# MohammadJohari/myslam

Hardware: AMD Instinct MI355X
Metric: ray.samples/s (render+bwd) (higher is better)
Workload: dtype f32; 1 GPU; BASELINE configs[1]: Replica room0 (synthetic), 4096 rays x 64 samples (56+8); mapping iteration: sample + render fwd + loss + bwd (planes+decoders), no optimiser; rays_of_the_job=4096, rays_this_rank=4096, samples_per_ray=64, plane_bytes=27147008, planes_layout=channels_last, parallelism=single GPU, launch=hipGraph replay of the captured iteration

## Files before the change

myslam_amd/csrc/eslam_scatter.hip:

```cpp
#include <mutex>
#include <type_traits>
#include "eslam_decode_tile.h"
#include "eslam_dec_reduce.h"
#include "eslam_ray_order_dev.h"

typedef float float2_t __attribute__((ext_vector_type(2)));

__global__ __launch_bounds__(1024) void ray_order_kernel(const float* __restrict__ rays_o,
                                                         const float* __restrict__ rays_d, int R,
                                                         int* __restrict__ perm, int key_bits, const int n_order,
                                                         float* __restrict__ clear, const long long clear_words) {
    extern __shared__ __attribute__((aligned(16))) unsigned hist[];
    if ((int)blockIdx.x >= n_order) {
        ray_clear_block(clear, clear_words, (int)blockIdx.x - n_order, (int)gridDim.x - n_order);
        return;
    }
    ray_order_block(rays_o, rays_d, R, perm, key_bits, (int)blockIdx.x, hist);
}

#define FIX_SCALE 17592186044416.0f
#define FIX_LIMIT 262144.0f
struct ShadowOff { int64_t o[NPL]; };
constexpr int SC_NT = 512;
constexpr int GZ_WP = 20;
template <bool RENDER, bool DET, int SPT = 4, bool GZ = false>
__global__ __launch_bounds__(SC_NT) void scatter_sort_kernel(const PlaneSet planes, const Bound bnd,
                                                          const float* __restrict__ rays_o,
                                                          const float* __restrict__ rays_d,
                                                          const float* __restrict__ z_vals,
                                                          const int* __restrict__ perm, int R, int S,
                                                          const float* __restrict__ g_feat, int bundle, int nbundles,
                                                          long long* __restrict__ shadow,
                                                          const ShadowOff shoff, const DecReduceArgs red, const int red_blocks,
                                                          const float* __restrict__ gz_w1_sdf, const float* __restrict__ gz_w1_rgb) {
    constexpr int NT = SC_NT;
    static_assert(!GZ || (RENDER && !DET), "GZ: the float render path only");
    constexpr int BM = SPT * NT;
    constexpr int CH = WAVE * SPT;
    static_assert(SPT == 2 || SPT == 4, "samples per thread");
    constexpr int SLOT_BITS = (BM == 1024) ? 10 : 11;
    constexpr unsigned SLOT_MASK = BM - 1;
    static_assert(BM == 1024 || BM == 2048, "bundle size");
    __shared__ __attribute__((aligned(16))) unsigned lds_raw[6 * BM];
    __shared__ __attribute__((aligned(16))) float gz_w[GZ ? ESLAM_C_DIM * GZ_WP : 4];
    __shared__ __attribute__((aligned(16))) float gz_a[GZ ? NT : 4];
    float4_t* const sw = (float4_t*)lds_raw;
    unsigned* const sxy = lds_raw + 4 * BM;
    int* const sgrow = (int*)(lds_raw + 5 * BM);
    unsigned* const cnt = lds_raw;
    unsigned* const swsum = lds_raw + 2 * BM;
    int* const sbox = (int*)(lds_raw + 2 * BM + 64);
    unsigned* const skey = lds_raw;
    unsigned* const txy = lds_raw + BM;
    float* const ttm = (float*)(lds_raw + 2 * BM + 128);
    float* const ttM = (float*)(lds_raw + 3 * BM + 128);
    int* const trow = (int*)(lds_raw + 4 * BM + 128);
    constexpr unsigned PAD_XY = 0xFFFFFFFFu;
    const int lane = threadIdx.x & 63, wave = threadIdx.x >> 6;
    const int hx = lane >> 5, c = lane & 31;

    if (red_blocks > 0 && (int)blockIdx.x < red_blocks) {
        if ((int)blockIdx.x < 2 * DEC_RED_COLBLOCKS)
            dec_grad_reduce_block<NT>(red, blockIdx.x % DEC_RED_COLBLOCKS, blockIdx.x / DEC_RED_COLBLOCKS, (float*)lds_raw);
        return;
    }
    const int bid = (int)blockIdx.x - red_blocks;
    bool plane_major = false;
    if (RENDER && perm) {
        const float* fan = (const float*)(perm + (size_t)ESLAM_RAY_ORDERS * R);
        const float f0 = fan[0], f1 = fan[1], f2 = fan[2];
        const float second = fmaxf(fminf(f0, f1), fminf(fmaxf(f0, f1), f2));
        plane_major = second >= 1.4f;
    }
    int bidx, pi;
    if (plane_major) { bidx = bid % nbundles; pi = bid / nbundles; }
    else { pi = bid % NPL; bidx = bid / NPL; }
    if (bidx >= nbundles || pi >= NPL) return;
    const int d = pi / 6, o = (pi % 6) >> 1, lvl = pi & 1;
    const eslam_plane_t& P = planes.p[pi];
    float gz_wv = 0.0f;
    if (GZ) gz_wv = (d ? gz_w1_rgb : gz_w1_sdf)[(threadIdx.x >> 5) * ESLAM_FEAT + lvl * ESLAM_C_DIM + (threadIdx.x & 31)];
    static_assert(!GZ || NT == ESLAM_HIDDEN * ESLAM_C_DIM, "one element of the slice per thread");
    const int pw = P.w, ph = P.h;
    const int psy = (int)P.stride_y, psx = (int)P.stride_x, psc = (int)P.stride_c;
    float* __restrict__ grad = P.grad;
    const int64_t npts = RENDER ? (int64_t)R * S : (int64_t)R;
    const int nunits = RENDER ? R : (int)((npts + 63) / 64);
    const int per = RENDER ? S : 64;
    const int u0 = bidx * bundle;
    const int nu = min(bundle, nunits - u0);
    const int n = nu * per;

    bool swap = false;
    if (threadIdx.x == 0) { sbox[0] = 0x7FFFFFFF; sbox[1] = -1; sbox[2] = 0x7FFFFFFF; sbox[3] = -1; }
    __syncthreads();

    AxisCoord cax[SPT], cay[SPT];
    int cpt[SPT];
    int bx0 = 0x7FFFFFFF, bx1 = -1, by0 = 0x7FFFFFFF, by1 = -1;
#pragma unroll
    for (int k = 0; k < SPT; ++k) {
        const int slot = threadIdx.x + k * NT;
        cpt[k] = -1;
        if (slot < n) {
            const int ui = u0 + slot / per, s = slot % per;
            const int unit = (RENDER && perm) ? perm[(size_t)o * R + ui] : ui;
            const int64_t pt = RENDER ? (int64_t)unit * S + s : (int64_t)unit * 64 + s;
            if (pt < npts) {
                float x, y, z;
                if (RENDER) {
                    const float zz = z_vals[pt];
                    x = rays_o[unit * 3 + 0] + rays_d[unit * 3 + 0] * zz;
                    y = rays_o[unit * 3 + 1] + rays_d[unit * 3 + 1] * zz;
                    z = rays_o[unit * 3 + 2] + rays_d[unit * 3 + 2] * zz;
                } else {
                    x = z_vals[pt * 3 + 0]; y = z_vals[pt * 3 + 1]; z = z_vals[pt * 3 + 2];
                }
                x = norm_coord(x, bnd.lo[0], bnd.hi[0]);
                y = norm_coord(y, bnd.lo[1], bnd.hi[1]);
                z = norm_coord(z, bnd.lo[2], bnd.hi[2]);
                cax[k] = axis_coord((o == 2) ? y : x, pw);
                cay[k] = axis_coord((o == 0) ? y : z, ph);
                cpt[k] = (int)pt;
                bx0 = min(bx0, cax[k].i0); bx1 = max(bx1, cax[k].i0);
                by0 = min(by0, cay[k].i0); by1 = max(by1, cay[k].i0);
            }
        }
    }
    if (GZ) gz_w[(threadIdx.x & 31) * GZ_WP + (threadIdx.x >> 5)] = gz_wv;
    bx0 = wave_min_i(bx0); bx1 = wave_max_i(bx1);
    by0 = wave_min_i(by0); by1 = wave_max_i(by1);
    if (lane == 0) {
        atomicMin(&sbox[0], bx0); atomicMax(&sbox[1], bx1);
        atomicMin(&sbox[2], by0); atomicMax(&sbox[3], by1);
    }
    __syncthreads();
    const int bxmin = sbox[0], bxmax = sbox[1], bymin = sbox[2], bymax = sbox[3];
    __syncthreads();
    if (bxmax < 0) return;
    swap = (bymax - bymin) > (bxmax - bxmin);
    const int mmin = swap ? bymin : bxmin, mext = (swap ? bymax : bxmax) - mmin + 2;
    const int Mmin = swap ? bxmin : bymin, Mext = (swap ? bxmax : bymax) - Mmin + 1;
    const bool counting = (int64_t)mext * Mext <= 4 * BM;
    if (counting) {
        constexpr int WPT = 2 * BM / NT;
        for (int i = threadIdx.x; i < 2 * BM; i += NT) cnt[i] = 0u;
        __syncthreads();
        unsigned loc[SPT], tick[SPT];
#pragma unroll
        for (int k = 0; k < SPT; ++k) {
            loc[k] = 0; tick[k] = 0;
            if (cpt[k] >= 0) {
                const int im = swap ? cay[k].i0 : cax[k].i0, iM = swap ? cax[k].i0 : cay[k].i0;
                loc[k] = (unsigned)((iM - Mmin) * mext + (im - mmin));
                const unsigned sh = (loc[k] & 1u) * 16u;
                tick[k] = (atomicAdd(&cnt[loc[k] >> 1], 1u << sh) >> sh) & 0xFFFFu;
            }
        }
        __syncthreads();
        unsigned w[WPT], local = 0;
#pragma unroll
        for (int j = 0; j < WPT; ++j) {
            w[j] = cnt[threadIdx.x * WPT + j];
            local += (w[j] & 0xFFFFu) + (w[j] >> 16);
        }
        const unsigned incl = wave_incl_sum_u(local);
        if (lane == WAVE - 1) swsum[wave] = incl;
        __syncthreads();
        unsigned run = incl - local, nvalid = 0;
        for (int wv = 0; wv < NT / WAVE; ++wv) {
            if (wv < wave) run += swsum[wv];
            nvalid += swsum[wv];
        }
#pragma unroll
        for (int j = 0; j < WPT; ++j) {
            const unsigned lo16 = w[j] & 0xFFFFu, hi16 = w[j] >> 16;
            cnt[threadIdx.x * WPT + j] = run | ((run + lo16) << 16);
            run += lo16 + hi16;
        }
        __syncthreads();
        unsigned pos[SPT];
#pragma unroll
        for (int k = 0; k < SPT; ++k) pos[k] = ((cnt[loc[k] >> 1] >> ((loc[k] & 1u) * 16u)) & 0xFFFFu) + tick[k];
        __syncthreads();
#pragma unroll
        for (int k = 0; k < SPT; ++k) {
            if (cpt[k] >= 0) {
                const AxisCoord& am = swap ? cay[k] : cax[k];
                const AxisCoord& aM = swap ? cax[k] : cay[k];
                const unsigned q = pos[k];
                sxy[q] = ((unsigned)(cay[k].i0 * psy + cax[k].i0 * psx) << 2) | (unsigned)(am.i1 > am.i0) |
                         ((unsigned)(aM.i1 > aM.i0) << 1);
                sw[q] = (float4_t){(1.0f - am.t) * (1.0f - aM.t), (1.0f - am.t) * aM.t, am.t * (1.0f - aM.t), am.t * aM.t};
                sgrow[q] = cpt[k];
            }
        }
        for (int i = (int)nvalid + threadIdx.x; i < BM; i += NT) {
            sxy[i] = PAD_XY;
            sw[i] = (float4_t){0.f, 0.f, 0.f, 0.f};
            sgrow[i] = 0;
        }
        __syncthreads();
    } else {
#pragma unroll
    for (int k = 0; k < SPT; ++k) {
        const int slot = threadIdx.x + k * NT;
        unsigned key = 0xFFFFFFFFu;
        if (cpt[k] >= 0) {
            const AxisCoord& am = swap ? cay[k] : cax[k];
            const AxisCoord& aM = swap ? cax[k] : cay[k];
            const int cell = aM.i0 * (swap ? ph : pw) + am.i0;
            key = ((unsigned)cell << SLOT_BITS) | (unsigned)slot;
            txy[slot] = ((unsigned)(cay[k].i0 * psy + cax[k].i0 * psx) << 2) | (unsigned)(am.i1 > am.i0) |
                        ((unsigned)(aM.i1 > aM.i0) << 1);
            ttm[slot] = am.t;
            ttM[slot] = aM.t;
            trow[slot] = cpt[k];
        }
        skey[slot] = key;
    }
    __syncthreads();

    {
        const int wbase = wave * CH;
        for (int k = 2; k <= BM; k <<= 1) {
            for (int j = k >> 1; j > 0; j >>= 1) {
                if (j >= CH) {
                    __syncthreads();
#pragma unroll
                    for (int t = 0; t < SPT / 2; ++t) {
                        const int p = threadIdx.x + t * NT;
                        const int i = ((p & ~(j - 1)) << 1) | (p & (j - 1));
                        const int l = i | j;
                        const unsigned a = skey[i], b2 = skey[l];
                        if ((a > b2) == ((i & k) == 0)) { skey[i] = b2; skey[l] = a; }
                    }
                    __syncthreads();
                } else {
#pragma unroll
                    for (int t = 0; t < SPT / 2; ++t) {
                        const int p = lane + t * WAVE;
                        const int i = wbase + (((p & ~(j - 1)) << 1) | (p & (j - 1)));
                        const int l = i | j;
                        const unsigned a = skey[i], b2 = skey[l];
                        if ((a > b2) == ((i & k) == 0)) { skey[i] = b2; skey[l] = a; }
                    }
                    WAVE_SYNC();
                }
            }
        }
    }
    __syncthreads();
    unsigned pxy[SPT];
    float ptm[SPT], ptM[SPT];
    int prow[SPT];
#pragma unroll
    for (int k = 0; k < SPT; ++k) {
        const unsigned key = skey[threadIdx.x + k * NT];
        const bool valid = key != 0xFFFFFFFFu;
        const int slot = key & SLOT_MASK;
        pxy[k] = valid ? txy[slot] : PAD_XY;
        ptm[k] = valid ? ttm[slot] : 0.f;
        ptM[k] = valid ? ttM[slot] : 0.f;
        prow[k] = valid ? trow[slot] : 0;
    }
    __syncthreads();
#pragma unroll
    for (int k = 0; k < SPT; ++k) {
        const int q = threadIdx.x + k * NT;
        const bool valid = pxy[k] != PAD_XY;
        sxy[q] = pxy[k];
        sw[q] = valid ? (float4_t){(1.0f - ptm[k]) * (1.0f - ptM[k]), (1.0f - ptm[k]) * ptM[k], ptm[k] * (1.0f - ptM[k]),
                                   ptm[k] * ptM[k]}
                      : (float4_t){0.f, 0.f, 0.f, 0.f};
        sgrow[q] = prow[k];
    }
    __syncthreads();
    }

    const char* __restrict__ gcol = GZ ? (const char*)(g_feat + (size_t)d * (size_t)npts * 16)
                                       : (const char*)(g_feat + d * 64 + lvl * 32);
    unsigned cur_xy = PAD_XY;
    unsigned last_xy = PAD_XY;
    typedef typename std::conditional<DET, long long, float>::type acc_t;
    acc_t acc0 = 0, acc1 = 0;
    bool det_bad = false;
    const int e0 = wave * CH;

    const unsigned lane_off = (unsigned)(c * psc) << 2;
    const unsigned dm_bytes = (unsigned)(swap ? psy : psx) << 2, dM_bytes = (unsigned)(swap ? psx : psy) << 2;
    char* __restrict__ gbytes = DET ? (char*)(shadow + shoff.o[pi]) : (char*)grad;
    float* const gz_as = gz_a + (GZ ? wave * WAVE : 0);
    auto flush = [&](bool lower_half_only) {
        if (cur_xy != PAD_XY) {
            acc_t f0 = acc0, f1 = acc1;
            if (GZ) {
                gz_as[lane] = (float)acc0;
                WAVE_SYNC();
                const float4_t* const A = (const float4_t*)(gz_as + hx * 32);
                unsigned wrow = (unsigned)(c * GZ_WP);
                asm volatile("" : "+v"(wrow));
                const float4_t* const Wc = (const float4_t*)(gz_w + wrow);
                float r0 = 0.0f, r1 = 0.0f;
#pragma unroll
                for (int jj = 0; jj < 4; ++jj) {
                    const float4_t a0 = A[jj], a1 = A[4 + jj], wv = Wc[jj];
#pragma unroll
                    for (int i = 0; i < 4; ++i) { r0 += wv[i] * a0[i]; r1 += wv[i] * a1[i]; }
                    if (jj & 1) asm volatile("" : "+v"(r0), "+v"(r1));
                }
                WAVE_SYNC();
                f0 = (acc_t)r0;
                f1 = (acc_t)r1;
            }
            const unsigned o0 = (cur_xy & ~3u) + lane_off + ((cur_xy & 1u) & (unsigned)hx) * dm_bytes;
            const unsigned o1 = o0 + ((cur_xy >> 1) & 1u) * dM_bytes;
            if (DET) {
                if (!lower_half_only || hx == 0) {
                    atomicAdd((unsigned long long*)(gbytes + 2 * (size_t)o0), (unsigned long long)f0);
                    atomicAdd((unsigned long long*)(gbytes + 2 * (size_t)o1), (unsigned long long)f1);
                    if (det_bad) {
                        atomicAdd((float*)((char*)grad + o0), __builtin_nanf(""));
                        atomicAdd((float*)((char*)grad + o1), __builtin_nanf(""));
                    }
                }
            } else if (!lower_half_only || hx == 0) {
                atomicAdd((float*)(gbytes + o0), (float)f0);
                atomicAdd((float*)(gbytes + o1), (float)f1);
            }
        }
    };

    struct Rec { unsigned xy; int row; unsigned long long fresh, adjacent; };
    auto fetch = [&](int blk, unsigned prev_last) {
        Rec r;
        const int e = e0 + blk * WAVE + lane;
        r.xy = sxy[e];
        r.row = sgrow[e] * (GZ ? 64 : 512);
        unsigned prev = __shfl_up(r.xy, 1, WAVE);
        if (lane == 0) prev = prev_last;
        const bool fresh = r.xy != prev;
        const bool adj = fresh && r.xy != PAD_XY && prev != PAD_XY && (prev & 1u) && (r.xy & ~3u) == (prev & ~3u) + dm_bytes;
        r.fresh = __ballot(fresh);
        r.adjacent = __ballot(adj);
        return r;
    };
    constexpr int WALK_N = 8;
    const float2_t* const wlane = (const float2_t*)sw + hx;
    const float* const wlane1 = (const float*)sw + (lane >> 4);
    const __amdgpu_buffer_rsrc_t grsrc = __builtin_amdgcn_make_buffer_rsrc((void*)gcol, 0, GZ ? (int)((unsigned)npts * 64u) : (int)((unsigned)npts * 512u - (unsigned)(d * 64 + lvl * 32) * 4u), 0x00020000);
    const int cvoff = GZ ? (lane & 15) * 4 : c * 4;
#define LOAD_HALF(buf, rec, half)                                                             \
    _Pragma("unroll") for (int t = 0; t < WALK_N; ++t) {                                      \
        const int rowb = __builtin_amdgcn_readlane((rec).row, (half) * WALK_N + t);           \
        buf[t] = __builtin_bit_cast(float, __builtin_amdgcn_raw_buffer_load_b32(grsrc, cvoff, rowb, 0)); \
    }
#define WALK_HALF(buf, rec, half, ebase)                                                      \
    _Pragma("unroll") for (int t = 0; t < WALK_N; ++t) {                                      \
        const int idx = (half) * WALK_N + t;                                                  \
        float2_t w2 = {0.f, 0.f};                                                             \
        if (GZ) w2[0] = wlane1[4 * ((ebase) + idx)];                                          \
        else w2 = wlane[2 * ((ebase) + idx)];                                                 \
        if (((idx < 32 ? fresh_lo : fresh_hi) >> (idx & 31)) & 1u) {      \
            if (((idx < 32 ? adj_lo : adj_hi) >> (idx & 31)) & 1u) {                          \
                 \
                flush(true);                                                                  \
                const acc_t s0 = __shfl_xor(acc0, 32, WAVE), s1 = __shfl_xor(acc1, 32, WAVE); \
                acc0 = hx ? (acc_t)0 : s0;                                                    \
                acc1 = (hx || GZ) ? (acc_t)0 : s1;                                            \
                if (DET) {             \
                    const int carried_bad = __shfl_xor((int)det_bad, 32, WAVE);               \
                    det_bad = !hx && carried_bad;                                             \
                }                                                                             \
            } else {                                                                          \
                flush(false);                                                                 \
                det_bad = false;                                                              \
                acc0 = 0;                                                                     \
                acc1 = 0;                                                                     \
            }                                                                                 \
            cur_xy = (unsigned)__builtin_amdgcn_readlane((int)(rec).xy, idx);                 \
        }                                                                                     \
        const float g = buf[t];         \
        if (DET) {                                                                            \
            const float t0_ = g * w2[0], t1_ = g * w2[1];                                     \
            det_bad = det_bad || !(fabsf(t0_) < FIX_LIMIT) || !(fabsf(t1_) < FIX_LIMIT);      \
            acc0 += (acc_t)__float2ll_rn(t0_ * FIX_SCALE);                                    \
            acc1 += (acc_t)__float2ll_rn(t1_ * FIX_SCALE);                                    \
        } else if (GZ) {                                                                      \
            acc0 += (acc_t)(g * w2[0]);                                                       \
        } else {                                                                              \
            acc0 += (acc_t)(g * w2[0]);                                                       \
            acc1 += (acc_t)(g * w2[1]);                                                       \
        }                                                                                     \
    }

    const int nblk = CH / WAVE;
    const int ngrp = WAVE / WALK_N;
    float ga[WALK_N], gb[WALK_N];
    Rec rec = fetch(0, PAD_XY);
    LOAD_HALF(ga, rec, 0)
#pragma unroll 1
    for (int blk = 0; blk < nblk; ++blk) {
        if ((unsigned)__builtin_amdgcn_readfirstlane((int)rec.xy) == PAD_XY) break;
        last_xy = (unsigned)__builtin_amdgcn_readlane((int)rec.xy, WAVE - 1);
        Rec nxt = rec;
        if (blk + 1 < nblk) nxt = fetch(blk + 1, last_xy);
        const int ebase = e0 + blk * WAVE;
        const unsigned fresh_lo = (unsigned)__builtin_amdgcn_readfirstlane((int)(unsigned)rec.fresh);
        const unsigned fresh_hi = (unsigned)__builtin_amdgcn_readfirstlane((int)(unsigned)(rec.fresh >> 32));
        const unsigned adj_lo = (unsigned)__builtin_amdgcn_readfirstlane((int)(unsigned)rec.adjacent);
        const unsigned adj_hi = (unsigned)__builtin_amdgcn_readfirstlane((int)(unsigned)(rec.adjacent >> 32));
#pragma unroll
        for (int g2 = 0; g2 < ngrp; g2 += 2) {
            LOAD_HALF(gb, rec, g2 + 1)
            WALK_HALF(ga, rec, g2, ebase)
            if (g2 + 2 < ngrp) {
                LOAD_HALF(ga, rec, g2 + 2)
            } else if (blk + 1 < nblk) {
                LOAD_HALF(ga, nxt, 0)
            }
            WALK_HALF(gb, rec, g2 + 1, ebase)
        }
        rec = nxt;
    }
#undef LOAD_HALF
#undef WALK_HALF
    flush(false);
}

__global__ __launch_bounds__(256) void scatter_fixed_to_float_kernel(float* __restrict__ grad, long long* __restrict__ shadow,
                                                                     int64_t n) {
    for (int64_t i = (int64_t)blockIdx.x * 256 + threadIdx.x; i < n; i += (int64_t)gridDim.x * 256) {
        const long long v = shadow[i];
        if (v != 0) {
            grad[i] += (float)((double)v * (1.0 / 17592186044416.0));
            shadow[i] = 0;
        }
    }
}

int eslam_scatter_v2_init();

static int ray_order_launch(const char* who, const float* rays_o, const float* rays_d, int R, int32_t* perm, void* clear,
                            int64_t clear_bytes, eslam_stream_t stream) {
    if (ray_order_check_args(who, rays_o, rays_d, R, perm, clear, clear_bytes)) return 1;
    if (R <= 0 && clear_bytes == 0) return 0;
    hipStream_t st = (hipStream_t)stream;
    if (int rc = eslam_scatter_v2_init()) return rc;
    const int key_bits = ray_order_key_bits(R);
    const int n_clear = ray_clear_blocks(clear_bytes);
    const int n_order = ray_order_blocks(R);
    hipLaunchKernelGGL(ray_order_kernel, dim3(n_order + n_clear), dim3(1024), ray_order_lds_bytes(key_bits), st,
                       rays_o, rays_d, R, perm, key_bits, n_order, (float*)clear, (long long)(clear_bytes >> 2));
    return eslam_check_launch("ray_order_kernel");
}

extern "C" int eslam_ray_order(const float* rays_o, const float* rays_d, int R, int32_t* perm, eslam_stream_t stream) {
    if (R <= 0) return 0;
    return ray_order_launch("eslam_ray_order", rays_o, rays_d, R, perm, nullptr, 0, stream);
}

extern "C" int eslam_ray_order_clear(const float* rays_o, const float* rays_d, int R, int32_t* perm, void* clear_ptr,
                                     int64_t clear_bytes, eslam_stream_t stream) {
    return ray_order_launch("eslam_ray_order_clear", rays_o, rays_d, R, perm, clear_ptr, clear_bytes, stream);
}

#define SC_SMALL_WGS 192
static int scatter_bundle_size(int per, int nunits, int* bm_out) {
    int bm = 2048;
    if (!eslam_deterministic()) {
        const int big = 2048 / per;
        const int nb = big > 0 ? (nunits + big - 1) / big : nunits;
        bm = (nb * NPL <= SC_SMALL_WGS && 1024 / per >= 1) ? 1024 : 2048;
    }
    *bm_out = bm;
    return bm / per;
}

extern "C" int eslam_scatter_bundle_samples(int64_t n, int S, int render) {
    if (n <= 0 || (render && (S <= 0 || S > 256))) return 0;
    int bm = 0;
    (void)scatter_bundle_size(render ? S : 64, render ? (int)n : (int)((n + 63) / 64), &bm);
    return bm;
}

bool eslam_scatter_can_reduce(bool render) {
    return render && !eslam_deterministic();
}

int eslam_scatter_v2(const eslam_plane_t* planes, const Bound& bnd, const float* rays_o, const float* rays_d,
                     const float* z_or_pts, int64_t R, int S, bool render, const float* g_feat, const int* perm,
                     hipStream_t st, const DecReduceArgs* red, const eslam_decoders_t* gz_dec) {
    PlaneSet ps;
    for (int i = 0; i < NPL; ++i) {
        ps.p[i] = planes[i];

    }
    const int64_t N = render ? R * S : R;
    const int nunits = render ? (int)R : (int)((N + 63) / 64);
    if (gz_dec && (!render || eslam_deterministic())) {
        eslam_set_error("scatter: the rank-16 path serves the float render mode only");
        return 1;
    }
    static_assert(2 * 64 <= 512 && ESLAM_HIDDEN * 4 == 64, "the rank-16 rows' offsets lie inside the N * 512 limit checked below");
    if (gz_dec && (N * 128 >= ((int64_t)1 << 32) - 256 || N * 64 > INT32_MAX)) {
        eslam_set_error("scatter: %lld points exceed the 32-bit offset range of the 16-wide gradient rows", (long long)N);
        return 1;
    }
    if (N * 512 >= ((int64_t)1 << 32)) {
        eslam_set_error("scatter: %lld points exceed the 32-bit offset range of the feature-gradient buffer (8.3 M): split "
                        "the batch", (long long)N);
        return 1;
    }
    for (int i = 0; i < NPL; ++i) {
        const int64_t extent = (ESLAM_C_DIM - 1) * planes[i].stride_c + (int64_t)(planes[i].h - 1) * planes[i].stride_y +
                               (int64_t)(planes[i].w - 1) * planes[i].stride_x + 1;
        if (extent >= ((int64_t)1 << 30)) {
            eslam_set_error("scatter: plane %d spans %lld elements, limit 2^30", i, (long long)extent);
            return 1;
        }
    }
    const int per = render ? S : 64;
    int bm;
    const int bundle = scatter_bundle_size(per, nunits, &bm);
    for (int i = 0; i < NPL; ++i)
        if ((int64_t)planes[i].w * planes[i].h >= ((1 << 21) - 2)) {
            eslam_set_error("scatter: plane %d has %d x %d cells, limit 2^21", i, planes[i].h, planes[i].w);
            return 1;
        }
    const int nbundles = (nunits + bundle - 1) / bundle;
    dim3 grid(nbundles * NPL);
    DecReduceArgs red_args = {};
    int red_blocks = 0;
    if (red) {
        if (!eslam_scatter_can_reduce(render)) {
            eslam_set_error("scatter: cannot carry the decoder-gradient reduction in this mode");
            return 1;
        }
        red_args = *red;
        red_blocks = (2 * DEC_RED_COLBLOCKS + 7) / 8 * 8;
        grid.x += red_blocks;
    }
#define LAUNCH_SC(RD, PERM, SS, ...)                                                                                      \
    hipLaunchKernelGGL((scatter_sort_kernel<RD, false, ##__VA_ARGS__>), grid, dim3(SC_NT), 0, st, ps, bnd, rays_o, rays_d, z_or_pts, \
                       PERM, (int)R, SS, g_feat, bundle, nbundles, (long long*)nullptr, ShadowOff{}, red_args, red_blocks, \
                       gz_dec ? gz_dec->w1 : nullptr, gz_dec ? gz_dec->cw1 : nullptr)
    if (eslam_deterministic()) {
        ShadowOff so;
        int64_t total = 0;
        for (int i = 0; i < NPL; ++i) {
            const int64_t numel = (int64_t)ESLAM_C_DIM * planes[i].h * planes[i].w;
            const int64_t extent = (ESLAM_C_DIM - 1) * planes[i].stride_c + (int64_t)(planes[i].h - 1) * planes[i].stride_y +
                                   (int64_t)(planes[i].w - 1) * planes[i].stride_x + 1;
            if (extent != numel) {
                eslam_set_error("scatter (deterministic mode): plane %d is not dense", i);
                return 1;
            }
            so.o[i] = total;
            total += numel;
        }
        constexpr int MAXDEV = 64;
        static long long* shadows[MAXDEV];
        static int64_t shadow_ns[MAXDEV];
        static std::mutex shadow_mu;
        int devi = 0;
        if (hipGetDevice(&devi) != hipSuccess || devi < 0 || devi >= MAXDEV) {
            eslam_set_error("scatter (deterministic mode): no usable current device");
            return 2;
        }
        long long* shadow;
        {
            std::lock_guard<std::mutex> lk(shadow_mu);
            if (shadow_ns[devi] < total) {
                hipStreamCaptureStatus cs = hipStreamCaptureStatusNone;
                (void)hipStreamIsCapturing(st, &cs);
                if (cs != hipStreamCaptureStatusNone) {
                    eslam_set_error("scatter (deterministic mode): run one eager iteration before capturing a graph");
                    return 1;
                }
                long long* fresh = nullptr;
                if (hipMalloc(&fresh, (size_t)total * 8) != hipSuccess || hipMemset(fresh, 0, (size_t)total * 8) != hipSuccess) {
                    eslam_set_error("scatter (deterministic mode): cannot allocate the %lld-element shadow", (long long)total);
                    return 2;
                }
                shadows[devi] = fresh;
                shadow_ns[devi] = total;
            }
            shadow = shadows[devi];
        }
        if (render)
            hipLaunchKernelGGL((scatter_sort_kernel<true, true>), grid, dim3(SC_NT), 0, st, ps, bnd, rays_o, rays_d,
                               z_or_pts, perm, (int)R, S, g_feat, bundle, nbundles, shadow, so, DecReduceArgs{}, 0, nullptr, nullptr);
        else
            hipLaunchKernelGGL((scatter_sort_kernel<false, true>), grid, dim3(SC_NT), 0, st, ps, bnd, rays_o, rays_d,
                               z_or_pts, (const int*)nullptr, (int)R, 64, g_feat, bundle, nbundles, shadow, so,
                               DecReduceArgs{}, 0, nullptr, nullptr);
        if (int rc = eslam_check_launch("scatter_sort_kernel<det>")) return rc;
        for (int i = 0; i < NPL; ++i) {
            const int64_t numel = (int64_t)ESLAM_C_DIM * planes[i].h * planes[i].w;
            hipLaunchKernelGGL(scatter_fixed_to_float_kernel, dim3((unsigned)((numel + 255) / 256 < 2048 ? (numel + 255) / 256 : 2048)),
                               dim3(256), 0, st, planes[i].grad, shadow + so.o[i], numel);
        }
        return eslam_check_launch("scatter_fixed_to_float_kernel");
    }
    if (gz_dec) {
        if (bm == 1024) LAUNCH_SC(true, perm, S, 2, true);
        else LAUNCH_SC(true, perm, S, 4, true);
    } else if (render) {
        if (bm == 1024) LAUNCH_SC(true, perm, S, 2);
        else LAUNCH_SC(true, perm, S);
    } else {
        if (bm == 1024) LAUNCH_SC(false, (const int*)nullptr, 64, 2);
        else LAUNCH_SC(false, (const int*)nullptr, 64);
    }
#undef LAUNCH_SC
    return eslam_check_launch("scatter_sort_kernel");
}

bool eslam_planes_channels_last(const eslam_plane_t* planes, int first, int count);
int eslam_validate_planes(const eslam_plane_t* planes, int first, int count);

int eslam_scatter_v2_init() {
    static bool done = false;
    if (done) return 0;
    if (hipFuncSetAttribute((const void*)ray_order_kernel, hipFuncAttributeMaxDynamicSharedMemorySize,
                            ORD_CELLS * (int)sizeof(unsigned)) != hipSuccess) {
        eslam_set_error("scatter: hipFuncSetAttribute(MaxDynamicSharedMemorySize) failed");
        return 2;
    }
    done = true;
    return 0;
}
```

Measured before the change: 1.138 billion ray.samples/s.

## Restructure GZ scatter walk to process four samples per step across lane quads

Adds a dedicated GZ path in the plane-gradient scatter kernel. Each lane group of 16 now handles one of four consecutive samples, with per-sample row indices and float4 corner weights. Partial sums are combined with permlane16/permlane32 swaps before the shared-memory projection and the atomics. The aim is to cut the number of serial walk steps and per-sample loads per wave in the compressed-gradient path, at the cost of more complex per-nibble cell-closing logic and reliance on gfx950 permlane-swap instructions.

```diff
diff --git a/myslam_amd/csrc/eslam_scatter.hip b/myslam_amd/csrc/eslam_scatter.hip
--- a/myslam_amd/csrc/eslam_scatter.hip
+++ b/myslam_amd/csrc/eslam_scatter.hip
@@ -291,28 +291,124 @@
     const unsigned dm_bytes = (unsigned)(swap ? psy : psx) << 2, dM_bytes = (unsigned)(swap ? psx : psy) << 2;
     char* __restrict__ gbytes = DET ? (char*)(shadow + shoff.o[pi]) : (char*)grad;
     float* const gz_as = gz_a + (GZ ? wave * WAVE : 0);
+    if constexpr (GZ) {
+        int wl = lane;
+        asm volatile("" : "+v"(wl));
+        const int s = wl >> 4, whx = wl >> 5, wc = wl & 31;
+        const unsigned wlane_off = (unsigned)(wc * psc) << 2;
+        const int up1 = ((wl + WAVE - 1) & (WAVE - 1)) << 2;
+        float2_t alo = {0.f, 0.f}, ahi = {0.f, 0.f};
+        auto flush4 = [&](const bool lower_half_only) {
+            if (cur_xy == PAD_XY) return;
+            float x0 = alo[0], y0 = alo[1], x1 = ahi[0], y1 = ahi[1];
+            asm volatile("s_nop 1\n\tv_permlane16_swap_b32 %0, %1" : "+v"(x0), "+v"(y0));
+            asm volatile("s_nop 1\n\tv_permlane16_swap_b32 %0, %1" : "+v"(x1), "+v"(y1));
+            float r0 = x0 + y0, r1 = x1 + y1;
+            asm volatile("s_nop 1\n\tv_permlane32_swap_b32 %0, %1" : "+v"(r0), "+v"(r1));
+            gz_as[wl] = r0 + r1;
+            WAVE_SYNC();
+            const float4_t* const A = (const float4_t*)(gz_as + whx * 32);
+            unsigned wrow = (unsigned)(wc * GZ_WP);
+            asm volatile("" : "+v"(wrow));
+            const float4_t* const Wc = (const float4_t*)(gz_w + wrow);
+            float f0 = 0.0f, f1 = 0.0f;
+#pragma unroll
+            for (int jj = 0; jj < 4; ++jj) {
+                const float4_t v0 = A[jj], v1 = A[4 + jj], wv = Wc[jj];
+#pragma unroll
+                for (int i = 0; i < 4; ++i) { f0 += wv[i] * v0[i]; f1 += wv[i] * v1[i]; }
+                if ((jj & 1) || SPT == 2) asm volatile("" : "+v"(f0), "+v"(f1));
+            }
+            WAVE_SYNC();
+            const unsigned o0 = (cur_xy & ~3u) + wlane_off + ((cur_xy & 1u) & (unsigned)whx) * dm_bytes;
+            const unsigned o1 = o0 + ((cur_xy >> 1) & 1u) * dM_bytes;
+            if (!lower_half_only || whx == 0) {
+                atomicAdd((float*)(gbytes + o0), f0);
+                atomicAdd((float*)(gbytes + o1), f1);
+            }
+        };
+        struct Rec4 { unsigned xy; unsigned long long fresh, adjacent; };
+        auto fetch4 = [&](int blk, unsigned prev_last) {
+            Rec4 r;
+            r.xy = sxy[e0 + blk * WAVE + wl];
+            unsigned prev = (unsigned)__builtin_amdgcn_ds_bpermute(up1, (int)r.xy);
+            if (wl == 0) prev = prev_last;
+            const bool fresh = r.xy != prev;
+            const bool adj = fresh && r.xy != PAD_XY && prev != PAD_XY && (prev & 1u) && (r.xy & ~3u) == (prev & ~3u) + dm_bytes;
+            r.fresh = __ballot(fresh);
+            r.adjacent = __ballot(adj);
+            return r;
+        };
+        auto close_cell = [&](const Rec4& rec, const int e, const int kk, const bool carry, const float4_t w4, float& g) {
+            const float gk = (s < kk) ? g : 0.f;
+            g = (s < kk) ? 0.f : g;
+            alo += gk * w4.xy;
+            ahi += gk * w4.zw;
+            flush4(carry);
+            alo = carry ? ahi : (float2_t){0.f, 0.f};
+            ahi = (float2_t){0.f, 0.f};
+            cur_xy = (unsigned)__builtin_amdgcn_readlane((int)rec.xy, e + kk);
+        };
+        constexpr int WALK_Q = 4;
+        const __amdgpu_buffer_rsrc_t grsrc4 = __builtin_amdgcn_make_buffer_rsrc((void*)gcol, 0, (int)((unsigned)npts * 64u), 0x00020000);
+        const int j4 = (wl & 15) * 4;
+        const int* const rlane = sgrow + s;
+        const float4_t* const wlane4 = sw + s;
+#define LOAD_Q(buf, eb, grp)                                                                  \
+    _Pragma("unroll") for (int t = 0; t < WALK_Q; ++t) {                                      \
+        const int row = rlane[(eb) + 4 * ((grp) * WALK_Q + t)];                               \
+        buf[t] = __builtin_bit_cast(float, __builtin_amdgcn_raw_buffer_load_b32(grsrc4, (row << 6) + j4, 0, 0)); \
+    }
+#define WALK_Q4(buf, rec, grp, eb)                                                            \
+    _Pragma("unroll") for (int t = 0; t < WALK_Q; ++t) {                                      \
+        const int st = (grp) * WALK_Q + t;                                                    \
+        const float4_t w4 = wlane4[(eb) + 4 * st];                                            \
+        const unsigned nib = ((st < 8 ? fresh_lo : fresh_hi) >> (4 * (st & 7))) & 15u;        \
+        float g = buf[t];                                                                     \
+        for (unsigned m = nib; __builtin_expect(m != 0u, 0); m &= m - 1u) {                   \
+            const int kk = __builtin_ctz(m);                                                  \
+            close_cell(rec, 4 * st, kk, ((st < 8 ? adj_lo : adj_hi) >> (4 * (st & 7) + kk)) & 1u, w4, g); \
+        }                                                                                     \
+        alo += g * w4.xy;            \
+        ahi += g * w4.zw;                                                                     \
+    }
+        constexpr int nblk = CH / WAVE;
+        constexpr int ngrp = WAVE / (4 * WALK_Q);
+        float ga[WALK_Q], gb[WALK_Q];
+        Rec4 rec = fetch4(0, PAD_XY);
+        LOAD_Q(ga, e0, 0)
+#pragma unroll 1
+        for (int blk = 0; blk < nblk; ++blk) {
+            if ((unsigned)__builtin_amdgcn_readfirstlane((int)rec.xy) == PAD_XY) break;
+            last_xy = (unsigned)__builtin_amdgcn_readlane((int)rec.xy, WAVE - 1);
+            Rec4 nxt = rec;
+            if (blk + 1 < nblk) nxt = fetch4(blk + 1, last_xy);
+            const int ebase = e0 + blk * WAVE;
+            const unsigned fresh_lo = (unsigned)__builtin_amdgcn_readfirstlane((int)(unsigned)rec.fresh);
+            const unsigned fresh_hi = (unsigned)__builtin_amdgcn_readfirstlane((int)(unsigned)(rec.fresh >> 32));
+            const unsigned adj_lo = (unsigned)__builtin_amdgcn_readfirstlane((int)(unsigned)rec.adjacent);
+            const unsigned adj_hi = (unsigned)__builtin_amdgcn_readfirstlane((int)(unsigned)(rec.adjacent >> 32));
+#pragma unroll
+            for (int g2 = 0; g2 < ngrp; g2 += 2) {
+                LOAD_Q(gb, ebase, g2 + 1)
+                WALK_Q4(ga, rec, g2, ebase)
+                if (g2 + 2 < ngrp) {
+                    LOAD_Q(ga, ebase, g2 + 2)
+                } else if (blk + 1 < nblk) {
+                    LOAD_Q(ga, ebase + WAVE, 0)
+                }
+                WALK_Q4(gb, rec, g2 + 1, ebase)
+            }
+            rec = nxt;
+        }
+#undef LOAD_Q
+#undef WALK_Q4
+        flush4(false);
+        return;
+    }
     auto flush = [&](bool lower_half_only) {
         if (cur_xy != PAD_XY) {
-            acc_t f0 = acc0, f1 = acc1;
-            if (GZ) {
-                gz_as[lane] = (float)acc0;
-                WAVE_SYNC();
-                const float4_t* const A = (const float4_t*)(gz_as + hx * 32);
-                unsigned wrow = (unsigned)(c * GZ_WP);
-                asm volatile("" : "+v"(wrow));
-                const float4_t* const Wc = (const float4_t*)(gz_w + wrow);
-                float r0 = 0.0f, r1 = 0.0f;
-#pragma unroll
-                for (int jj = 0; jj < 4; ++jj) {
-                    const float4_t a0 = A[jj], a1 = A[4 + jj], wv = Wc[jj];
-#pragma unroll
-                    for (int i = 0; i < 4; ++i) { r0 += wv[i] * a0[i]; r1 += wv[i] * a1[i]; }
-                    if (jj & 1) asm volatile("" : "+v"(r0), "+v"(r1));
-                }
-                WAVE_SYNC();
-                f0 = (acc_t)r0;
-                f1 = (acc_t)r1;
-            }
+            const acc_t f0 = acc0, f1 = acc1;
             const unsigned o0 = (cur_xy & ~3u) + lane_off + ((cur_xy & 1u) & (unsigned)hx) * dm_bytes;
             const unsigned o1 = o0 + ((cur_xy >> 1) & 1u) * dM_bytes;
             if (DET) {
@@ -336,7 +432,7 @@
         Rec r;
         const int e = e0 + blk * WAVE + lane;
         r.xy = sxy[e];
-        r.row = sgrow[e] * (GZ ? 64 : 512);
+        r.row = sgrow[e] * 512;
         unsigned prev = __shfl_up(r.xy, 1, WAVE);
         if (lane == 0) prev = prev_last;
         const bool fresh = r.xy != prev;
@@ -347,9 +443,8 @@
     };
     constexpr int WALK_N = 8;
     const float2_t* const wlane = (const float2_t*)sw + hx;
-    const float* const wlane1 = (const float*)sw + (lane >> 4);
-    const __amdgpu_buffer_rsrc_t grsrc = __builtin_amdgcn_make_buffer_rsrc((void*)gcol, 0, GZ ? (int)((unsigned)npts * 64u) : (int)((unsigned)npts * 512u - (unsigned)(d * 64 + lvl * 32) * 4u), 0x00020000);
-    const int cvoff = GZ ? (lane & 15) * 4 : c * 4;
+    const __amdgpu_buffer_rsrc_t grsrc = __builtin_amdgcn_make_buffer_rsrc((void*)gcol, 0, (int)((unsigned)npts * 512u - (unsigned)(d * 64 + lvl * 32) * 4u), 0x00020000);
+    const int cvoff = c * 4;
 #define LOAD_HALF(buf, rec, half)                                                             \
     _Pragma("unroll") for (int t = 0; t < WALK_N; ++t) {                                      \
         const int rowb = __builtin_amdgcn_readlane((rec).row, (half) * WALK_N + t);           \
@@ -358,16 +453,14 @@
 #define WALK_HALF(buf, rec, half, ebase)                                                      \
     _Pragma("unroll") for (int t = 0; t < WALK_N; ++t) {                                      \
         const int idx = (half) * WALK_N + t;                                                  \
-        float2_t w2 = {0.f, 0.f};                                                             \
-        if (GZ) w2[0] = wlane1[4 * ((ebase) + idx)];                                          \
-        else w2 = wlane[2 * ((ebase) + idx)];                                                 \
+        const float2_t w2 = wlane[2 * ((ebase) + idx)];                                       \
         if (((idx < 32 ? fresh_lo : fresh_hi) >> (idx & 31)) & 1u) {      \
             if (((idx < 32 ? adj_lo : adj_hi) >> (idx & 31)) & 1u) {                          \
                  \
                 flush(true);                                                                  \
                 const acc_t s0 = __shfl_xor(acc0, 32, WAVE), s1 = __shfl_xor(acc1, 32, WAVE); \
                 acc0 = hx ? (acc_t)0 : s0;                                                    \
-                acc1 = (hx || GZ) ? (acc_t)0 : s1;                                            \
+                acc1 = hx ? (acc_t)0 : s1;                                                    \
                 if (DET) {             \
                     const int carried_bad = __shfl_xor((int)det_bad, 32, WAVE);               \
                     det_bad = !hx && carried_bad;                                             \
@@ -386,8 +479,6 @@
             det_bad = det_bad || !(fabsf(t0_) < FIX_LIMIT) || !(fabsf(t1_) < FIX_LIMIT);      \
             acc0 += (acc_t)__float2ll_rn(t0_ * FIX_SCALE);                                    \
             acc1 += (acc_t)__float2ll_rn(t1_ * FIX_SCALE);                                    \
-        } else if (GZ) {                                                                      \
-            acc0 += (acc_t)(g * w2[0]);                                                       \
         } else {                                                                              \
             acc0 += (acc_t)(g * w2[0]);                                                       \
             acc1 += (acc_t)(g * w2[1]);                                                       \
```

After: 1.205 billion ray.samples/s (median of 6 runs). 5.8% higher.
